# mapillary/OpenSfM

Measured on AMD Instinct MI355X. Metric: image-pairs matched/sec (+ BA LM-iters/sec, 5k cams / 500k pts), higher is better.
Workload: dtype i8 (exact int32 accumulate) + f64 RANSAC

## Files before the change

### opensfm_amd/csrc/match.hip

```cpp
#include <algorithm>
#include <cstdlib>
#include <type_traits>

#include "osfm_internal.h"

typedef int v4i __attribute__((ext_vector_type(4)));
typedef int v16i __attribute__((ext_vector_type(16)));

#ifdef OSFM_DBG_PHASES
__device__ unsigned long long g_phase[22];
#define OSFM_TICK(var) const unsigned long long var = wall_clock64();
#define OSFM_PHASE(i, t0, t1) if (threadIdx.x == 0) atomicAdd(&g_phase[i], (t1) - (t0));
extern "C" int osfm_dbg_phases(unsigned long long *out, int reset) {
  if (hipMemcpyFromSymbol(out, HIP_SYMBOL(g_phase), sizeof(g_phase)) != hipSuccess) return 1;
  if (reset) {
    unsigned long long z[22] = {};
    if (hipMemcpyToSymbol(HIP_SYMBOL(g_phase), z, sizeof(z)) != hipSuccess) return 1;
  }
  return 0;
}
#else
#define OSFM_TICK(var)
#define OSFM_PHASE(i, t0, t1)
#endif

namespace {

constexpr int kThreads = 256;
constexpr int kWaves = 4;
constexpr int kRT = 2;
constexpr int kNone = 0xFFFF;
constexpr int kCollisionD2 = 1 << 22;

__device__ __forceinline__ bool ratio_ok(int d1sq, int d2sq, double ratio) {
  if (ratio < 0.0) return (float)d1sq < (float)(-ratio) * (float)d2sq;
  const float f1 = sqrtf((float)d1sq), f2 = sqrtf((float)d2sq);
  return (double)f1 < ratio * (double)f2;
}

__device__ __forceinline__ long xcd_remap(long b, long n) {
  const long q = n >> 3, r = n & 7;
  const long xcd = b & 7, within = b >> 3;
  return (xcd < r ? xcd * (q + 1) : r * (q + 1) + (xcd - r) * q) + within;
}

struct MatchArgs {
  const int8_t *tiles;
  const int32_t *norms;
  const int32_t *hneg;
  const float *descf;
  const float *qerr;
  const int64_t *tile_off;
  const int32_t *counts;
  const int32_t *pairs;
  long n_pairs;
  double ratio;
  int symmetric;
  int query_second;
  int cap;
  int ncap;
  int32_t *out_counts;
  uint32_t *out_matches;
  int32_t *out_flags;
  long pad_tile;
  const uint32_t *bin;
  const float *seg;
  int32_t *tickets;
};
constexpr int kTicketStride = 32;

__device__ __forceinline__ void emit_matches(const MatchArgs &a, long p, int nC, const int *colBI,
                                             const unsigned short *rowres, int *misc, int tid, bool swap_halves) {
  const int lane = tid & 63, w = tid >> 6;
  int base = 0;
  for (int j0 = 0; j0 < nC; j0 += kThreads) {
    const int j = j0 + tid;
    bool m = false;
    int r = kNone;
    if (j < nC) {
      r = colBI[j];
      m = (r != kNone) && (!a.symmetric || rowres[r] == j);
    }
    const unsigned long long bal = __ballot(m);
    const int prefix = __popcll(bal & ((1ull << lane) - 1ull));
    if (lane == 0) misc[w] = __popcll(bal);
    __syncthreads();
    int woff = 0, total = 0;
#pragma unroll
    for (int w2 = 0; w2 < kWaves; ++w2) {
      const int cnt = misc[w2];
      woff += (w2 < w) ? cnt : 0;
      total += cnt;
    }
    if (m) {
      const int k = base + woff + prefix;
      if (k < a.cap) a.out_matches[p * a.cap + k] = swap_halves ? ((uint32_t)r | ((uint32_t)j << 16)) : ((uint32_t)j | ((uint32_t)r << 16));
    }
    base += total;
    __syncthreads();
  }
  if (tid == 0) a.out_counts[p] = base;
}

__device__ __forceinline__ int dot_rows8(const int8_t *tilesA, int rowA, const int8_t *tilesB, int rowB) {
  const int8_t *pa = tilesA + (long)(rowA >> 5) * OSFM_TILE_BYTES + (rowA & 31) * 16;
  const int8_t *pb = tilesB + (long)(rowB >> 5) * OSFM_TILE_BYTES + (rowB & 31) * 16;
  v4i av[8], bv[8];
#pragma unroll
  for (int q = 0; q < 8; ++q) {
    av[q] = *(const v4i *)(pa + q * 512);
    bv[q] = *(const v4i *)(pb + q * 512);
  }
  int s0 = 0, s1 = 0;
#pragma unroll
  for (int q = 0; q < 8; q += 2)
#pragma unroll
    for (int e = 0; e < 4; ++e) {
      s0 = __builtin_amdgcn_sdot4(av[q][e], bv[q][e], s0, false);
      s1 = __builtin_amdgcn_sdot4(av[q + 1][e], bv[q + 1][e], s1, false);
    }
  return s0 + s1;
}

template <class P>
__device__ __forceinline__ P *uniform_ptr(P *p) {
  const unsigned long long v = (unsigned long long)p;
  const unsigned lo = __builtin_amdgcn_readfirstlane((unsigned)v), hi = __builtin_amdgcn_readfirstlane((unsigned)(v >> 32));
  return (P *)(((unsigned long long)hi << 32) | lo);
}

__device__ __forceinline__ int wave_max(int v) {
#pragma unroll
  for (int m = 32; m >= 1; m >>= 1) v = max(v, __shfl_xor(v, m));
  return v;
}

__device__ __forceinline__ int row16_max(int x) {
  x = max(x, __builtin_amdgcn_update_dpp(x, x, 0xB1, 0xF, 0xF, false));
  x = max(x, __builtin_amdgcn_update_dpp(x, x, 0x4E, 0xF, 0xF, false));
  x = max(x, __builtin_amdgcn_update_dpp(x, x, 0x141, 0xF, 0xF, false));
  x = max(x, __builtin_amdgcn_update_dpp(x, x, 0x140, 0xF, 0xF, false));
  return x;
}

constexpr double kFqSlack = 8e-6;
__device__ __forceinline__ double fq_ratio(double ratio) { return ratio < 0.0 ? sqrt(-ratio) : ratio; }
__device__ __forceinline__ bool fq_surely_fails(int d0lo_sq, int d1hi_sq, double eps, double r) {
  const double D0lo = fmax(sqrt((double)max(d0lo_sq, 0)) - eps, 0.0) * (1.0 - kFqSlack);
  const double D1hi = (sqrt((double)max(d1hi_sq, 0)) + eps) * (1.0 + kFqSlack);
  return D0lo >= r * D1hi;
}
__device__ __forceinline__ bool fq_surely_passes(int d0hi_sq, int d1lo_sq, double eps, double r) {
  const double D0hi = (sqrt((double)max(d0hi_sq, 0)) + eps) * (1.0 + kFqSlack);
  const double D1lo = fmax(sqrt((double)max(d1lo_sq, 0)) - eps, 0.0) * (1.0 - kFqSlack);
  return D0hi < r * D1lo && D0hi < D1lo;
}
__device__ __forceinline__ float wave_minf(float v) {
#pragma unroll
  for (int m = 32; m >= 1; m >>= 1) v = fminf(v, __shfl_xor(v, m));
  return v;
}

constexpr int kCT4 = 8;
constexpr int kChunkCols4 = kCT4 * 32;
constexpr int kChunkBytes4 = kCT4 * OSFM_TILE_BYTES;

struct QueryPassShared {
  unsigned char *bbuf;
  int *hbuf;
};

template <bool GATHER, bool FQ, class Hooks>
__device__ __forceinline__ int query_pass(const QueryPassShared &sh, const int8_t *tilesQ, const int32_t *normQ, int nQ, int nslots,
                                          const unsigned short *qsel, const int8_t *tilesT, const int32_t *normT, const int32_t *hnegT,
                                          int nT, const int8_t *tiles_pad, const int32_t *hneg_pad, unsigned short *out, double ratio,
                                          int tid, const float *descQ, const float *descT, double eps, int *hit_word, int &any_hit,
                                          Hooks &&hooks) {
  asm volatile("" : "+v"(tid));
  asm volatile("" : "+s"(ratio));
  const int lane = tid & 63;
  const int w = __builtin_amdgcn_readfirstlane(tid >> 6);
  const int tT = (nT + 31) >> 5;
  const int tS = (nslots + 31) >> 5;
  const int nchunks = (tS + kCT4 - 1) / kCT4;
  const int nrb = (tT + kWaves * kRT - 1) / (kWaves * kRT);
  int flag = 0, hit = 0;

  auto dma_chunk = [&](int c) {
    unsigned char *dst = sh.bbuf + (c & 1) * kChunkBytes4;
#pragma unroll
    for (int q = 0; q < kCT4; ++q) {
      const int gt = c * kCT4 + q;
      const int8_t *src;
      if (GATHER) {
        const int slot = gt * 32 + (lane & 31);
        const int f = slot < nslots ? (int)qsel[slot] : 0;
        src = tilesQ + (long)(f >> 5) * OSFM_TILE_BYTES + w * 1024 + (lane >> 5) * 512 + (f & 31) * 16;
      } else {
        src = tilesQ + (long)(gt < tS ? gt : 0) * OSFM_TILE_BYTES + tid * 16;
      }
      __builtin_amdgcn_global_load_lds((const __attribute__((address_space(1))) void *)src,
                                       (__attribute__((address_space(3))) void *)(dst + q * OSFM_TILE_BYTES + w * 1024), 16, 0, 0);
    }
  };

  auto load_seeds = [&](int rb, int slot) {
    const int t = rb * (kWaves * kRT) + w * kRT;
    const int32_t *h0 = uniform_ptr((t < tT) ? hnegT + (long)t * 32 : hneg_pad);
    const int32_t *h1 = uniform_ptr((t + 1 < tT) ? hnegT + (long)(t + 1) * 32 : hneg_pad);
    const int32_t *hp = ((lane >> 5) ? h1 : h0) + (lane & 31);
    __builtin_amdgcn_global_load_lds((const __attribute__((address_space(1))) void *)hp,
                                     (__attribute__((address_space(3))) void *)(sh.hbuf + slot * 256 + w * 64), 4, 0, 0);
  };
  auto load_rows = [&](int rb, v4i (&af)[kRT][4], int rt) {
    const int t = rb * (kWaves * kRT) + w * kRT + rt;
    const auto *tp = (const __attribute__((address_space(1))) int8_t *)uniform_ptr((t < tT) ? tilesT + (long)t * OSFM_TILE_BYTES : tiles_pad);
#pragma unroll
    for (int ks = 0; ks < 4; ++ks) af[rt][ks] = *(const __attribute__((address_space(1))) v4i *)(tp + ks * 1024 + lane * 16);
  };
  auto load_targets = [&](int rb, v4i (&af)[kRT][4], int slot) {
    load_seeds(rb, slot);
    load_rows(rb, af, 0);
    load_rows(rb, af, 1);
  };
  v16i hn[kRT];
  auto read_seeds_rt = [&](int slot, int rt) {
#pragma unroll
    for (int g = 0; g < 4; ++g) {
      const v4i hv = *(const v4i *)(sh.hbuf + slot * 256 + w * 64 + rt * 32 + 8 * g + 4 * (lane >> 5));
      hn[rt][4 * g + 0] = hv[0];
      hn[rt][4 * g + 1] = hv[1];
      hn[rt][4 * g + 2] = hv[2];
      hn[rt][4 * g + 3] = hv[3];
    }
  };
  auto read_seeds = [&](int slot) {
    read_seeds_rt(slot, 0);
    read_seeds_rt(slot, 1);
  };

  int cb[kCT4], cs[kCT4], ci[kCT4];
  const unsigned char *bb = sh.bbuf;
  v4i bf[4];

#define OSFM_TREE_A(X, A, B)             \
  A = max(max(X[0], X[1]), X[2]);        \
  B = max(max(X[8], X[9]), X[10]);
#define OSFM_TREE_B(X, A, B)             \
  A = max(max(A, X[3]), X[4]);           \
  B = max(max(B, X[11]), X[12]);
#define OSFM_TREE_C(X, A, B)             \
  A = max(max(A, X[5]), X[6]);           \
  B = max(max(B, X[13]), X[14]);
#define OSFM_TREE_D(X, A, B, M)          \
  M = max(max(A, B), X[7]);              \
  M = max(M, X[15]);
#define OSFM_PIN __builtin_amdgcn_sched_barrier(0);

  auto step = [&](const v4i (&af)[kRT][4], v4i (&nxt)[kRT][4], int rb, int rbn, int next_slot, int t0, const unsigned char *bq) {
    const int vrb = rb;
    v16i T[3];
    int mp = 0;
    asm volatile("; osfm-step: a step of the sweep begins (tests/test_kernel_budgets_sweep.py)");
#pragma unroll
    for (int t = 0; t < kCT4; ++t) {
      if (t == 0 && t0 > 0) {
        load_targets(rbn, nxt, next_slot);
        continue;
      }
      if (t < kCT4 - 1 && t < t0) continue;
      const unsigned char *nb = (t == kCT4 - 1 ? bq + t0 * OSFM_TILE_BYTES : bq + (t + 1) * OSFM_TILE_BYTES) + lane * 16;
      v16i &C1 = T[(2 * t) % 3];
      v16i &C2 = T[(2 * t + 1) % 3];
      v16i &P2 = T[(2 * t + 2) % 3];
      int a0 = 0, b0 = 0, a1 = 0, b1 = 0, m2 = 0;
      C1 = __builtin_amdgcn_mfma_i32_32x32x32_i8(af[0][0], bf[0], hn[0], 0, 0, 0);
      OSFM_PIN
      if (t > 0) {
        OSFM_TREE_A(C2, a0, b0)
        OSFM_TREE_B(C2, a0, b0)
        OSFM_TREE_C(C2, a0, b0)
        OSFM_TREE_D(C2, a0, b0, mp)
      } else {
        load_seeds(rbn, next_slot);
      }
      OSFM_PIN
      C2 = __builtin_amdgcn_mfma_i32_32x32x32_i8(af[1][0], bf[0], hn[1], 0, 0, 0);
      OSFM_PIN
      if (t == kCT4 - 1) {
        __builtin_amdgcn_s_waitcnt(0x0F70 | (2 * kRT * 4));
        read_seeds_rt(next_slot, 0);
      }
      bf[0] = *(const v4i *)(nb);
      if (t > 0) { OSFM_TREE_A(P2, a1, b1) }
      OSFM_PIN
      C1 = __builtin_amdgcn_mfma_i32_32x32x32_i8(af[0][1], bf[1], C1, 0, 0, 0);
      OSFM_PIN
      if (t > 0) { OSFM_TREE_B(P2, a1, b1) } else { load_rows(rbn, nxt, 0); }
      if (t == kCT4 - 1) read_seeds_rt(next_slot, 1);
      OSFM_PIN
      C2 = __builtin_amdgcn_mfma_i32_32x32x32_i8(af[1][1], bf[1], C2, 0, 0, 0);
      OSFM_PIN
      bf[1] = *(const v4i *)(nb + 1024);
      if (t > 0) { OSFM_TREE_C(P2, a1, b1) }
      OSFM_PIN
      C1 = __builtin_amdgcn_mfma_i32_32x32x32_i8(af[0][2], bf[2], C1, 0, 0, 0);
      OSFM_PIN
      if (t > 0) { OSFM_TREE_D(P2, a1, b1, m2) } else { load_rows(rbn, nxt, 1); }
      OSFM_PIN
      C2 = __builtin_amdgcn_mfma_i32_32x32x32_i8(af[1][2], bf[2], C2, 0, 0, 0);
      OSFM_PIN
      bf[2] = *(const v4i *)(nb + 2048);
      if (t > 0) {
        m2 = max(m2, mp);
        asm("v_med3_i32 %0, %1, %2, %3" : "=v"(cs[t - 1]) : "v"(cb[t - 1]), "v"(m2), "v"(cs[t - 1]));
      }
      OSFM_PIN
      C1 = __builtin_amdgcn_mfma_i32_32x32x32_i8(af[0][3], bf[3], C1, 0, 0, 0);
      OSFM_PIN
      if (t > 0)
        asm volatile("v_cmp_gt_i32 vcc, %1, %2\n\ts_nop 1\n\tv_cndmask_b32 %0, %0, %3, vcc" : "+v"(ci[t - 1]) : "v"(m2), "v"(cb[t - 1]), "v"(vrb) : "vcc");
      OSFM_PIN
      C2 = __builtin_amdgcn_mfma_i32_32x32x32_i8(af[1][3], bf[3], C2, 0, 0, 0);
      OSFM_PIN
      bf[3] = *(const v4i *)(nb + 3072);
      if (t > 0) cb[t - 1] = max(cb[t - 1], m2);
      OSFM_PIN
    }
    {
      v16i &Q1 = T[(2 * (kCT4 - 1)) % 3];
      v16i &Q2 = T[(2 * (kCT4 - 1) + 1) % 3];
      int a0, b0, a1, b1, m1, m2;
      OSFM_TREE_A(Q1, a0, b0)
      OSFM_TREE_B(Q1, a0, b0)
      OSFM_TREE_C(Q1, a0, b0)
      OSFM_TREE_D(Q1, a0, b0, m1)
      OSFM_TREE_A(Q2, a1, b1)
      OSFM_TREE_B(Q2, a1, b1)
      OSFM_TREE_C(Q2, a1, b1)
      OSFM_TREE_D(Q2, a1, b1, m2)
      m2 = max(m2, m1);
      asm("v_med3_i32 %0, %1, %2, %3" : "=v"(cs[kCT4 - 1]) : "v"(cb[kCT4 - 1]), "v"(m2), "v"(cs[kCT4 - 1]));
      ci[kCT4 - 1] = m2 > cb[kCT4 - 1] ? rb : ci[kCT4 - 1];
      cb[kCT4 - 1] = max(cb[kCT4 - 1], m2);
    }
  };

  auto load_norm = [&](int c) {
    const int slot = c * kChunkCols4 + tid;
    const int f = slot < nslots ? (GATHER ? (int)qsel[slot] : slot) : -1;
    return (f >= 0 && f < nQ) ? normQ[f] : OSFM_PAD_NORM;
  };
  dma_chunk(0);
  v4i afA[kRT][4], afB[kRT][4];
  load_targets(0, afA, 0);
  int myna_next = load_norm(0);
  hooks.cold_issue();
  __builtin_amdgcn_s_waitcnt(0x0F70);
  hooks.cold_done();
  read_seeds(0);
  int sidx = 0;

  for (int c = 0; c < nchunks; ++c) {
    const int myslot = c * kChunkCols4 + tid;
    const int myf = myslot < nslots ? (GATHER ? (int)qsel[myslot] : myslot) : -1;
    const int myna = myna_next;
    __builtin_amdgcn_s_waitcnt(0x0F70);
    __syncthreads();
    bb = sh.bbuf + (c & 1) * kChunkBytes4;
    const int t0 = kCT4 - min(kCT4, tS - c * kCT4);
#pragma unroll
    for (int ks = 0; ks < 4; ++ks) bf[ks] = *(const v4i *)(bb + ks * 1024 + lane * 16);
#pragma unroll
    for (int t = 0; t < kCT4; ++t) {
      cb[t] = INT_MIN;
      cs[t] = INT_MIN;
      ci[t] = 0;
    }

    auto one_step = [&](const v4i (&cur)[kRT][4], v4i (&nxt)[kRT][4], int rb) {
      const int rbn = (rb + 1 < nrb) ? rb + 1 : 0;
      const bool live = rb * (kWaves * kRT) + w * kRT < tT;
      const int nslot = (sidx + 1) & 1;
      if (live) {
        step(cur, nxt, rb, rbn, nslot, t0, bb - t0 * OSFM_TILE_BYTES);
      } else {
        load_targets(rbn, nxt, nslot);
        __builtin_amdgcn_s_waitcnt(0x0F70);
        read_seeds(nslot);
      }
      ++sidx;
    };
    OSFM_TICK(tk0)
    hooks.chunk(c);
    if (c + 1 < nchunks) dma_chunk(c + 1);
    int rb = 0;
    for (; rb + 1 < nrb; rb += 2) {
      one_step(afA, afB, rb);
      one_step(afB, afA, rb + 1);
    }
    if (rb < nrb) {
      one_step(afA, afB, rb);
#pragma unroll
      for (int rt = 0; rt < kRT; ++rt)
#pragma unroll
        for (int ks = 0; ks < 4; ++ks) afA[rt][ks] = afB[rt][ks];
    }

    OSFM_TICK(tk1)
    if (c + 1 < nchunks) myna_next = load_norm(c + 1);
    __syncthreads();
    OSFM_TICK(tk2)
    int *scr = (int *)(sh.bbuf + (c & 1) * kChunkBytes4);
    {
      const int part = w * 2 + (lane >> 5);
#pragma unroll
      for (int t = 0; t < kCT4; ++t) {
        const int qt = (t - t0) & (kCT4 - 1);
        scr[(part * 3 + 0) * kChunkCols4 + qt * 32 + (lane & 31)] = cb[t];
        scr[(part * 3 + 1) * kChunkCols4 + qt * 32 + (lane & 31)] = cs[t];
        scr[(part * 3 + 2) * kChunkCols4 + qt * 32 + (lane & 31)] = ci[t];
      }
    }
    __syncthreads();
    int b = INT_MIN, s2 = INT_MIN, id = 0;
#pragma unroll
    for (int part = 0; part < 2 * kWaves; ++part) {
      const int pb = scr[(part * 3 + 0) * kChunkCols4 + tid], ps = scr[(part * 3 + 1) * kChunkCols4 + tid];
      const int pi = scr[(part * 3 + 2) * kChunkCols4 + tid];
      s2 = max(max(s2, ps), min(b, pb));
      id = pb > b ? (pi * 8 + part) : id;
      b = max(b, pb);
    }
    __syncthreads();
    bool want = false;
    if (myf >= 0 && myf < nQ) {
      const int d1lo = max(myna - (2 * b + 1), 0), d2hi = myna - 2 * s2;
      if (FQ) {
        want = !fq_surely_fails(d1lo, d2hi, eps, fq_ratio(ratio));
      } else {
        if (d2hi >= kCollisionD2 && ratio >= 0.0) flag = 1;
        want = ratio_ok(d1lo, d2hi, ratio);
      }
#ifdef OSFM_DBG_NORECHECK
      want = false;
#endif
      if (!want) out[myf] = kNone;
    }
    unsigned long long pending = __ballot(want);
    unsigned long long redo = 0;
    OSFM_TICK(tk3)
#ifdef OSFM_DBG_PHASES
    if (tid == 0) atomicAdd(&g_phase[(GATHER ? 5 : 0) + 4], (unsigned long long)__popcll(pending));
#endif
    while (pending) {
      int srcs[4];
#pragma unroll
      for (int g = 0; g < 4; ++g) {
        srcs[g] = pending ? (int)__builtin_ctzll(pending) : -1;
        pending &= pending - 1;
      }
      const int g = lane >> 4, sl = lane & 15;
      const int src = g == 0 ? srcs[0] : g == 1 ? srcs[1] : g == 2 ? srcs[2] : srcs[3];
      const int ssrc = src < 0 ? 0 : src;
      const int qf = __shfl(myf, ssrc), qna = __shfl(myna, ssrc), qb = __shfl(b, ssrc), qs = __shfl(s2, ssrc), qid = __shfl(id, ssrc);
      const bool tie = (qs == qb);
      const int qrb = qid >> 3, qw = (qid >> 1) & 3, qh = qid & 1;
      const int row0 = (qrb * (kWaves * kRT) + qw * kRT) * 32 + (sl & 3) + 8 * (sl >> 2) + 4 * qh, row1 = row0 + 32;
      int k0 = INT_MIN, k1 = INT_MIN;
      if (src >= 0 && !tie) {
        const bool ok0 = row0 < nT, ok1 = row1 < nT;
        const int r0 = ok0 ? row0 : 0, r1 = ok1 ? row1 : 0;
        const int8_t *pa = tilesQ + (long)(qf >> 5) * OSFM_TILE_BYTES + (qf & 31) * 16;
        const int8_t *p0 = tilesT + (long)(r0 >> 5) * OSFM_TILE_BYTES + (r0 & 31) * 16;
        const int8_t *p1 = tilesT + (long)(r1 >> 5) * OSFM_TILE_BYTES + (r1 & 31) * 16;
        v4i av[8], bv0[8], bv1[8];
#pragma unroll
        for (int q = 0; q < 8; ++q) {
          av[q] = *(const v4i *)(pa + q * 512);
          bv0[q] = *(const v4i *)(p0 + q * 512);
          bv1[q] = *(const v4i *)(p1 + q * 512);
        }
        const int n0 = normT[r0], n1 = normT[r1];
        int s0 = 0, s1 = 0;
#pragma unroll
        for (int q = 0; q < 8; ++q)
#pragma unroll
          for (int e = 0; e < 4; ++e) {
            s0 = __builtin_amdgcn_sdot4(av[q][e], bv0[q][e], s0, false);
            s1 = __builtin_amdgcn_sdot4(av[q][e], bv1[q][e], s1, false);
          }
        if (ok0) k0 = (2 * s0 - n0) * 32 + (31 - sl);
        if (ok1) k1 = (2 * s1 - n1) * 32 + (15 - sl);
      }
      const int kmax = row16_max(max(k0, k1));
      const int ksec = row16_max(k0 == kmax ? k1 : (k1 == kmax ? k0 : max(k0, k1)));
      if (src >= 0) {
        bool full = tie;
        int win = kNone;
        if (!tie) {
          const int m1 = kmax >> 5, ord = 31 - (kmax & 31);
          const int jwin = (qrb * (kWaves * kRT) + qw * kRT + (ord >> 4)) * 32 + (ord & 3) + 8 * ((ord & 15) >> 2) + 4 * qh;
          const int m2 = ksec >> 5;
          const int sa = max(m2, 2 * qs), sb = max(m2, 2 * qs + 1);
          if (FQ) {
            const double r = fq_ratio(ratio);
            if (fq_surely_passes(qna - m1, qna - sb, eps, r))
              win = jwin;
            else if (!fq_surely_fails(qna - m1, qna - sa, eps, r))
              full = true;
          } else {
            const bool ra = ratio_ok(qna - m1, qna - sa, ratio), rbb = ratio_ok(qna - m1, qna - sb, ratio);
            if (ra == rbb)
              win = ra ? jwin : kNone;
            else
              full = true;
          }
        }
        if (sl == 0 && !full) out[qf] = (unsigned short)win;
        hit |= (!full && win != kNone);
        redo |= (full && sl == 0) ? (1ull << src) : 0ull;
      }
    }
    OSFM_TICK(tk4)
    OSFM_PHASE((GATHER ? 5 : 0) + 0, tk0, tk1)
    OSFM_PHASE((GATHER ? 5 : 0) + 1, tk1, tk2)
    OSFM_PHASE((GATHER ? 5 : 0) + 2, tk2, tk3)
    OSFM_PHASE((GATHER ? 5 : 0) + 3, tk3, tk4)
    {
      unsigned lo = (unsigned)redo, hi = (unsigned)(redo >> 32);
#pragma unroll
      for (int m = 32; m >= 16; m >>= 1) {
        lo |= (unsigned)__shfl_xor((int)lo, m);
        hi |= (unsigned)__shfl_xor((int)hi, m);
      }
      redo = ((unsigned long long)(unsigned)__builtin_amdgcn_readfirstlane((int)hi) << 32) | (unsigned)__builtin_amdgcn_readfirstlane((int)lo);
    }
    if (FQ) flag += __popcll(redo);
    while (FQ && redo) {
      const int src = __builtin_ctzll(redo);
      redo &= redo - 1;
      const int qf = __shfl(myf, src), qna = __shfl(myna, src), qs2 = __shfl(s2, src);
      const double T = (sqrt((double)max(qna - 2 * qs2, 0)) + 2.0 * eps) * (1.0 + 4.0 * kFqSlack) + 1e-6;
      const double T2 = T * T;
      const int vthr = T2 >= 2.0e9 ? INT_MIN : qna - (int)T2 - 1;
      const float *qrow = descQ + (long)qf * OSFM_DESC_DIM;
      float bd0 = INFINITY, bd1 = INFINITY;
      int bi0 = INT_MAX;
      for (int i = lane; i < nT; i += 64) {
        const int v = 2 * dot_rows8(tilesQ, qf, tilesT, i) - normT[i];
        if (v >= vthr) {
          const float sq = l2sqr_rows_f32(qrow, descT + (long)i * OSFM_DESC_DIM);
          const float d = ratio < 0.0 ? sq : sqrtf(sq);
          if (d < bd1) {
            if (bd0 > d) {
              bd1 = bd0;
              bd0 = d;
              bi0 = i;
            } else {
              bd1 = d;
            }
          }
        }
      }
      const float m = wave_minf(bd0);
      const int jwin = -wave_max(bd0 == m ? -bi0 : INT_MIN);
      const float sec = wave_minf(bi0 == jwin ? bd1 : bd0);
      const bool ok = ratio < 0.0 ? (m < (float)(-ratio) * sec) : ((double)m < ratio * (double)sec);
      if (lane == 0) out[qf] = (unsigned short)(ok ? jwin : kNone);
      hit |= ok;
    }
    while (!FQ && redo) {
      const int src = __builtin_ctzll(redo);
      redo &= redo - 1;
      const int qf = __shfl(myf, src), qna = __shfl(myna, src);
      int lv = INT_MIN, lj = INT_MAX, ls = INT_MIN;
      for (int i = lane; i < nT; i += 64) {
        const int v = 2 * dot_rows8(tilesQ, qf, tilesT, i) - normT[i];
        ls = max(ls, min(lv, v));
        if (v > lv) {
          lv = v;
          lj = i;
        }
      }
      const int m1 = wave_max(lv);
      const int jwin = -wave_max(lv == m1 ? -lj : INT_MIN);
      const int m2 = wave_max(lj == jwin ? ls : lv);
      const bool ok = ratio_ok(qna - m1, qna - m2, ratio);
      if (lane == 0) out[qf] = (unsigned short)(ok ? jwin : kNone);
      hit |= ok;
    }
  }
  if (hit) *hit_word = 1;
  __syncthreads();
  any_hit = *hit_word;
  return flag;
}

struct PairRange {
  long first;
  int len;
};
__device__ __forceinline__ PairRange pair_range(long n_pairs, int x) {
  const long q = n_pairs >> 3, r = n_pairs & 7;
  return PairRange{x < r ? x * (q + 1) : r * (q + 1) + (x - r) * q, (int)(q + (x < r ? 1 : 0))};
}
__device__ __forceinline__ int draw_pair(const MatchArgs &a, int xcd, int *hdr, bool have, int t) {
  for (int k = hdr[8]; k < 8; ++k) {
    const int x = (xcd + k) & 7;
    const PairRange r = pair_range(a.n_pairs, x);
    if (!have) t = atomicAdd(a.tickets + x * kTicketStride, 1);
    have = false;
    if (t < r.len) {
      hdr[8] = k;
      return (int)(r.first + t);
    }
  }
  hdr[8] = 8;
  return -1;
}
__device__ __forceinline__ void finish_pair_header(const MatchArgs &a, int *hdr) {
  const int img1 = hdr[1], img2 = hdr[2];
  const int n1 = a.counts[img1], n2 = a.counts[img2];
  const int o1 = (int)a.tile_off[img1], o2 = (int)a.tile_off[img2];
  hdr[3] = n1;
  hdr[4] = n2;
  hdr[5] = o1;
  hdr[6] = o2;
  hdr[7] = 1;
}
__device__ __forceinline__ void fetch_pair_header(const MatchArgs &a, int xcd, int *hdr) {
  const int p = draw_pair(a, xcd, hdr, false, 0);
  hdr[0] = p;
  hdr[7] = 1;
  if (p >= 0) {
    const int img1 = a.pairs[2 * (long)p], img2 = a.pairs[2 * (long)p + 1];
    hdr[1] = img1;
    hdr[2] = img2;
    finish_pair_header(a, hdr);
  }
}
struct NextPairFetch {
  const MatchArgs &a;
  int xcd;
  int *hdr;
  int tid;
  int t;
  __device__ __forceinline__ void cold_issue() {
    if (tid == 0) {
      const int k = hdr[8];
      t = k < 8 ? atomicAdd(a.tickets + ((xcd + k) & 7) * kTicketStride, 1) : 0;
    }
  }
  __device__ __forceinline__ void cold_done() {
    if (tid == 0) {
      hdr[0] = draw_pair(a, xcd, hdr, hdr[8] < 8, t);
      hdr[7] = 0;
    }
  }
  __device__ __forceinline__ void chunk(int c) {
    if (c > 1 || __builtin_amdgcn_readfirstlane(tid >> 6) != 0) return;
    const int pn = __builtin_amdgcn_readfirstlane(hdr[0]);
    if (pn < 0) return;
    if (c == 0) {
      if (tid < 2)
        __builtin_amdgcn_global_load_lds((const __attribute__((address_space(1))) void *)(a.pairs + 2 * (long)pn + tid),
                                         (__attribute__((address_space(3))) void *)(hdr + 1), 4, 0, 0);
    } else if (tid < 4) {
      const int img = hdr[1 + (tid & 1)];
      const int32_t *src = tid < 2 ? a.counts + img : (const int32_t *)(a.tile_off + img);
      __builtin_amdgcn_global_load_lds((const __attribute__((address_space(1))) void *)src,
                                       (__attribute__((address_space(3))) void *)(hdr + 3), 4, 0, 0);
      if (tid == 0) hdr[7] = 1;
    }
  }
};
struct NoFetch {
  __device__ __forceinline__ void cold_issue() {}
  __device__ __forceinline__ void cold_done() {}
  __device__ __forceinline__ void chunk(int) {}
};

__device__ __forceinline__ int fresh_tid(int wave) {
  int t = wave * 64 + (int)__builtin_amdgcn_mbcnt_hi(~0u, __builtin_amdgcn_mbcnt_lo(~0u, 0u));
  asm volatile("" : "+v"(t));
  return t;
}

template <bool FQ>
__global__ void __launch_bounds__(kThreads, 2) match_fused_kernel(MatchArgs a) {
  extern __shared__ __attribute__((aligned(16))) unsigned char smem[];
  QueryPassShared sh;
  sh.bbuf = smem;
  sh.hbuf = (int *)(smem + 2 * kChunkBytes4);
  int *misc = (int *)(smem + 2 * kChunkBytes4) + 2 * kChunkCols4;
  int *hdr = misc + 16;
  unsigned short *resA = (unsigned short *)(hdr + 16);
  unsigned short *resB = resA + a.ncap;
  unsigned short *cand = resB + a.ncap;

  const int xcd = blockIdx.x & 7;
  const int8_t *tiles_pad = a.tiles + a.pad_tile * OSFM_TILE_BYTES;
  const int32_t *hneg_pad = a.hneg + a.pad_tile * 32;
  OSFM_TICK(tw0)
#ifdef OSFM_DBG_PHASES
  unsigned long long t_prev = tw0;
#endif
  const int wave = __builtin_amdgcn_readfirstlane(threadIdx.x >> 6);
  if (threadIdx.x == 0) {
    hdr[8] = 0;
    fetch_pair_header(a, xcd, hdr);
  }
  __syncthreads();
  for (;;) {
  const int tid = fresh_tid(wave);
  const long p = __builtin_amdgcn_readfirstlane(hdr[0]);
  if (p < 0) break;
  if (__builtin_amdgcn_readfirstlane(hdr[7]) == 0) {
    __syncthreads();
    if (tid == 0) finish_pair_header(a, hdr);
    __syncthreads();
  }
  const int img1 = __builtin_amdgcn_readfirstlane(hdr[1]), img2 = __builtin_amdgcn_readfirstlane(hdr[2]);
  const int n1 = __builtin_amdgcn_readfirstlane(hdr[3]), n2 = __builtin_amdgcn_readfirstlane(hdr[4]);
  const long off1 = __builtin_amdgcn_readfirstlane(hdr[5]), off2 = __builtin_amdgcn_readfirstlane(hdr[6]);
  if (tid == 0) {
    misc[8] = 0;
    misc[9] = 0;
    misc[10] = 0;
  }
  __syncthreads();
  if (n1 < 2 || n2 < 2) {
    if (tid == 0) {
      a.out_counts[p] = 0;
      a.out_flags[p] = 0;
      fetch_pair_header(a, xcd, hdr);
    }
    __syncthreads();
#ifdef OSFM_DBG_PHASES
    {
      OSFM_TICK(te)
      OSFM_PHASE(19, t_prev, te)
      if (threadIdx.x == 0) atomicAdd(&g_phase[20], 1ull);
      t_prev = te;
    }
#endif
    continue;
  }
  const bool rows_second = a.symmetric || a.query_second;
  const int imgA = rows_second ? img2 : img1, imgB = rows_second ? img1 : img2;
  const int nA = rows_second ? n2 : n1, nB = rows_second ? n1 : n2;
  const long offA = rows_second ? off2 : off1, offB = rows_second ? off1 : off2;
  const int8_t *tilesA = a.tiles + offA * OSFM_TILE_BYTES;
  const int8_t *tilesB = a.tiles + offB * OSFM_TILE_BYTES;
  const int32_t *normA = a.norms + offA * 32;
  const int32_t *normB = a.norms + offB * 32;
  const int32_t *hnegA = a.hneg + offA * 32;
  const int32_t *hnegB = a.hneg + offB * 32;
  OSFM_TICK(tq0)
  const float *descA = FQ ? a.descf + offA * (long)(32 * OSFM_DESC_DIM) : nullptr;
  const float *descB = FQ ? a.descf + offB * (long)(32 * OSFM_DESC_DIM) : nullptr;
  const double eps = FQ ? (double)a.qerr[imgA] + (double)a.qerr[imgB] : 0.0;
  int any = 0;
  auto flush_flag = [&](int f) {
    if (FQ) {
      if ((fresh_tid(wave) & 63) == 0 && f) atomicAdd(&misc[8], f);
    } else if (f) {
      misc[8] = 1;
    }
  };
  int flag = query_pass<false, FQ>(sh, tilesA, normA, nA, nA, nullptr, tilesB, normB, hnegB, nB, tiles_pad, hneg_pad, resA, a.ratio, fresh_tid(wave),
                                   descA, descB, eps, misc + 9, any, NextPairFetch{a, xcd, hdr, fresh_tid(wave), 0});
  OSFM_TICK(tq1)
  OSFM_PHASE(10, tq0, tq1)
  if (a.symmetric && any) {
    const int tid = fresh_tid(wave), lane = tid & 63, w = tid >> 6;
    for (int j = tid; j < nB; j += kThreads) resB[j] = kNone;
    __syncthreads();
    for (int q = tid; q < nA; q += kThreads) {
      const int b = resA[q];
      if (b != kNone) resB[b] = 0;
    }
    __syncthreads();
    int base = 0;
    for (int j0 = 0; j0 < nB; j0 += kThreads) {
      const int j = j0 + tid;
      const bool m = j < nB && resB[j] == 0;
      const unsigned long long bal = __ballot(m);
      if (lane == 0) misc[w] = __popcll(bal);
      __syncthreads();
      int woff = 0, total = 0;
#pragma unroll
      for (int w2 = 0; w2 < kWaves; ++w2) {
        const int cnt = misc[w2];
        woff += (w2 < w) ? cnt : 0;
        total += cnt;
      }
      if (m) {
        cand[base + woff + __popcll(bal & ((1ull << lane) - 1ull))] = (unsigned short)j;
        resB[j] = kNone;
      }
      base += total;
      __syncthreads();
    }
    const int nK = base;
    OSFM_TICK(tq2)
    OSFM_PHASE(11, tq1, tq2)
    flush_flag(flag);
    flag = query_pass<true, FQ>(sh, tilesB, normB, nB, nK, cand, tilesA, normA, hnegA, nA, tiles_pad, hneg_pad, resB, a.ratio, fresh_tid(wave), descB, descA,
                                 eps, misc + 10, any, NoFetch{});
  }
  OSFM_TICK(tq3)
  OSFM_PHASE(12, tq1, tq3)
  flush_flag(flag);
  __builtin_amdgcn_s_waitcnt(0x0F70);
  __syncthreads();
  if (fresh_tid(wave) == 0) a.out_flags[p] = misc[8];
  if (!any) {
    if (fresh_tid(wave) == 0) a.out_counts[p] = 0;
  } else {
    const int tid = fresh_tid(wave), lane = tid & 63, w = tid >> 6;
    const bool qs = !a.symmetric && a.query_second;
    const unsigned short *res1 = a.symmetric ? resB : resA;
    const unsigned short *res2 = a.symmetric ? resA : nullptr;
    const int nE = qs ? n2 : n1;
    int base = 0;
    for (int j0 = 0; j0 < nE; j0 += kThreads) {
      const int j = j0 + tid;
      bool m = false;
      int r = kNone;
      if (j < nE) {
        r = res1[j];
        m = (r != kNone) && (!res2 || res2[r] == j);
      }
      const unsigned long long bal = __ballot(m);
      const int prefix = __popcll(bal & ((1ull << lane) - 1ull));
      if (lane == 0) misc[w] = __popcll(bal);
      __syncthreads();
      int woff = 0, total = 0;
#pragma unroll
      for (int w2 = 0; w2 < kWaves; ++w2) {
        const int cnt = misc[w2];
        woff += (w2 < w) ? cnt : 0;
        total += cnt;
      }
      if (m) {
        const int k = base + woff + prefix;
        if (k < a.cap) a.out_matches[p * a.cap + k] = qs ? ((uint32_t)r | ((uint32_t)j << 16)) : ((uint32_t)j | ((uint32_t)r << 16));
      }
      base += total;
      __syncthreads();
    }
    if (tid == 0) a.out_counts[p] = base;
  }
  OSFM_TICK(tq4)
  OSFM_PHASE(13, tq3, tq4)
  OSFM_PHASE(14, tq0, tq4)
#ifdef OSFM_DBG_PHASES
  if (threadIdx.x == 0) atomicAdd(&g_phase[15], 1ull);
  OSFM_PHASE(16, t_prev, tq0)
  t_prev = tq4;
#endif
  }
#ifdef OSFM_DBG_PHASES
  if (threadIdx.x == 0) {
    atomicAdd(&g_phase[17], wall_clock64() - tw0);
    atomicAdd(&g_phase[18], 1ull);
  }
#endif
}

__device__ __forceinline__ void load_row(const int8_t *tiles, int row, v4i out[8]) {
  const int8_t *t = tiles + (long)(row >> 5) * OSFM_TILE_BYTES + (row & 31) * 16;
#pragma unroll
  for (int ks = 0; ks < 4; ++ks) {
    out[2 * ks] = *(const v4i *)(t + ks * 1024);
    out[2 * ks + 1] = *(const v4i *)(t + ks * 1024 + 512);
  }
}

__device__ void exact_direction(const int8_t *tilesQ, const int32_t *normQ, int nQ, const int8_t *tilesT,
                                const int32_t *normT, int nT, double ratio, int tid, int *res_int,
                                unsigned short *res_u16, const float *segQ, const float *segT) {
  for (int q = tid; q < nQ; q += kThreads) {
    v4i qa[8];
    load_row(tilesQ, q, qa);
    const int nq = normQ[q];
    const float sq = segQ ? segQ[q] : 0.f;
    float bd0 = INFINITY, bd1 = INFINITY;
    int bi0 = kNone;
    for (int t = 0; t < nT; ++t) {
      v4i ta[8];
      load_row(tilesT, t, ta);
      int sdot = 0;
#pragma unroll
      for (int k = 0; k < 8; ++k)
#pragma unroll
        for (int e = 0; e < 4; ++e) sdot = __builtin_amdgcn_sdot4(qa[k][e], ta[k][e], sdot, false);
      const int d2i = nq + normT[t] - 2 * sdot;
      float d2f = (float)d2i;
      if (segQ) {
        const float ts = sq - segT[t];
        const float tt = ts * ts;
        d2f = d2f + tt;
      }
      const float d = ratio < 0.0 ? d2f : sqrtf(d2f);
      if (d < bd1) {
        if (bd0 > d) {
          bd1 = bd0;
          bd0 = d;
          bi0 = t;
        } else {
          bd1 = d;
        }
      }
    }
    const bool ok = ratio < 0.0 ? (bd0 < (float)(-ratio) * bd1) : ((double)bd0 < ratio * (double)bd1);
    const int v = ok ? bi0 : kNone;
    if (res_int) res_int[q] = v;
    if (res_u16) res_u16[q] = (unsigned short)v;
  }
}

__global__ void __launch_bounds__(kThreads) match_exact_kernel(MatchArgs a, int only_flagged) {
  extern __shared__ __attribute__((aligned(16))) unsigned char smem[];
  int *colBI = (int *)smem;
  unsigned short *rowres = (unsigned short *)(colBI + a.ncap);
  int *misc = (int *)(rowres + a.ncap);
  const int tid = threadIdx.x;
  const long p = blockIdx.x;
  if (only_flagged && a.out_flags[p] == 0) return;
  const bool qs = !a.symmetric && a.query_second;
  const int imgC = a.pairs[2 * p + (qs ? 1 : 0)], imgR = a.pairs[2 * p + (qs ? 0 : 1)];
  const int nC = a.counts[imgC], nR = a.counts[imgR];
  if (nC < 2 || nR < 2) {
    if (tid == 0) a.out_counts[p] = 0;
    return;
  }
  const int8_t *tilesC = a.tiles + a.tile_off[imgC] * OSFM_TILE_BYTES;
  const int8_t *tilesR = a.tiles + a.tile_off[imgR] * OSFM_TILE_BYTES;
  const int32_t *normC = a.norms + a.tile_off[imgC] * 32;
  const int32_t *normR = a.norms + a.tile_off[imgR] * 32;
  const float *segC = a.seg ? a.seg + a.tile_off[imgC] * 32 : nullptr, *segR = a.seg ? a.seg + a.tile_off[imgR] * 32 : nullptr;
  exact_direction(tilesC, normC, nC, tilesR, normR, nR, a.ratio, tid, colBI, nullptr, segC, segR);
  if (a.symmetric) exact_direction(tilesR, normR, nR, tilesC, normC, nC, a.ratio, tid, nullptr, rowres, segR, segC);
  __syncthreads();
  emit_matches(a, p, nC, colBI, rowres, misc, tid, qs);
}

constexpr int kFloatTileFloats = 32 * OSFM_DESC_DIM;

__device__ void float_direction(const float *descQ, int nQ, const float *descT, int nT, double ratio, int tid, float *stage, int *res_int,
                                unsigned short *res_u16) {
  const int tT = (nT + 31) >> 5;
  for (int q0 = 0; q0 < nQ; q0 += kThreads) {
    const int q = q0 + tid;
    const bool live = q < nQ;
    float qa[OSFM_DESC_DIM];
#pragma unroll
    for (int k4 = 0; k4 < OSFM_DESC_DIM; k4 += 4) {
      float4 v = make_float4(0.f, 0.f, 0.f, 0.f);
      if (live) v = *(const float4 *)(descQ + (size_t)q * OSFM_DESC_DIM + k4);
      qa[k4] = v.x;
      qa[k4 + 1] = v.y;
      qa[k4 + 2] = v.z;
      qa[k4 + 3] = v.w;
    }
    float bd0 = INFINITY, bd1 = INFINITY;
    int bi0 = kNone;
    for (int tt = 0; tt < tT; ++tt) {
      __syncthreads();
      for (int k = tid * 4; k < kFloatTileFloats; k += kThreads * 4) *(float4 *)(stage + k) = *(const float4 *)(descT + (size_t)tt * kFloatTileFloats + k);
      __syncthreads();
      const int nt = min(32, nT - tt * 32);
      for (int t = 0; t < nt; ++t) {
        const float *b = stage + t * OSFM_DESC_DIM;
        float acc[4][8];
#pragma unroll
        for (int v = 0; v < 4; ++v)
#pragma unroll
          for (int l = 0; l < 8; ++l) acc[v][l] = 0.f;
#pragma unroll
        for (int jb = 0; jb < OSFM_DESC_DIM; jb += 32)
#pragma unroll
          for (int v = 0; v < 4; ++v)
#pragma unroll
            for (int l4 = 0; l4 < 8; l4 += 4) {
              const float4 c = *(const float4 *)(b + jb + 8 * v + l4);
              const float cc[4] = {c.x, c.y, c.z, c.w};
#pragma unroll
              for (int e = 0; e < 4; ++e) {
                const float d = qa[jb + 8 * v + l4 + e] - cc[e];
                const float sq = d * d;
                acc[v][l4 + e] = acc[v][l4 + e] + sq;
              }
            }
        float sv[8];
#pragma unroll
        for (int l = 0; l < 8; ++l) sv[l] = (acc[0][l] + acc[1][l]) + (acc[2][l] + acc[3][l]);
        const float sqd = ((sv[0] + sv[1]) + (sv[2] + sv[3])) + ((sv[4] + sv[5]) + (sv[6] + sv[7]));
        const float d = ratio < 0.0 ? sqd : sqrtf(sqd);
        if (d < bd1) {
          if (bd0 > d) {
            bd1 = bd0;
            bd0 = d;
            bi0 = tt * 32 + t;
          } else {
            bd1 = d;
          }
        }
      }
    }
    if (live) {
      const bool ok = ratio < 0.0 ? (bd0 < (float)(-ratio) * bd1) : ((double)bd0 < ratio * (double)bd1);
      const int v = ok ? bi0 : kNone;
      if (res_int) res_int[q] = v;
      if (res_u16) res_u16[q] = (unsigned short)v;
    }
  }
}

__global__ void __launch_bounds__(kThreads) match_float_kernel(MatchArgs a) {
  extern __shared__ __attribute__((aligned(16))) unsigned char smem[];
  float *stage = (float *)smem;
  int *colBI = (int *)(stage + kFloatTileFloats);
  unsigned short *rowres = (unsigned short *)(colBI + a.ncap);
  int *misc = (int *)(rowres + a.ncap);
  const int tid = threadIdx.x;
  const long p = blockIdx.x;
  if (tid == 0 && a.out_flags) a.out_flags[p] = 0;
  const bool qs = !a.symmetric && a.query_second;
  const int imgC = a.pairs[2 * p + (qs ? 1 : 0)], imgR = a.pairs[2 * p + (qs ? 0 : 1)];
  const int nC = a.counts[imgC], nR = a.counts[imgR];
  if (nC < 2 || nR < 2) {
    if (tid == 0) a.out_counts[p] = 0;
    return;
  }
  const float *descC = a.descf + a.tile_off[imgC] * kFloatTileFloats;
  const float *descR = a.descf + a.tile_off[imgR] * kFloatTileFloats;
  float_direction(descC, nC, descR, nR, a.ratio, tid, stage, colBI, nullptr);
  if (a.symmetric) float_direction(descR, nR, descC, nC, a.ratio, tid, stage, nullptr, rowres);
  __syncthreads();
  emit_matches(a, p, nC, colBI, rowres, misc, tid, qs);
}

constexpr int kHamStageRows = 256;

__device__ void hamming_direction(const uint32_t *binQ, int nQ, const uint32_t *binT, int nT, double ratio, int tid, uint32_t *stage, int *res_int,
                                  unsigned short *res_u16) {
  for (int q0 = 0; q0 < nQ; q0 += kThreads) {
    const int q = q0 + tid;
    const bool live = q < nQ;
    uint4 qa[4];
#pragma unroll
    for (int k = 0; k < 4; ++k) qa[k] = live ? *(const uint4 *)(binQ + (size_t)q * 16 + 4 * k) : make_uint4(0u, 0u, 0u, 0u);
    int bd0 = 0x7fffffff, bd1 = 0x7fffffff, bi0 = kNone;
    for (int t0 = 0; t0 < nT; t0 += kHamStageRows) {
      const int nt = min(kHamStageRows, nT - t0);
      __syncthreads();
      for (int k = tid; k < nt * 4; k += kThreads) *(uint4 *)(stage + 4 * k) = *(const uint4 *)(binT + (size_t)t0 * 16 + 4 * k);
      __syncthreads();
      for (int t = 0; t < nt; ++t) {
        const uint4 *b = (const uint4 *)(stage + t * 16);
        int d = 0;
#pragma unroll
        for (int k = 0; k < 4; ++k) {
          const uint4 c = b[k];
          d += __popc(qa[k].x ^ c.x) + __popc(qa[k].y ^ c.y) + __popc(qa[k].z ^ c.z) + __popc(qa[k].w ^ c.w);
        }
        if (d < bd1) {
          if (bd0 > d) {
            bd1 = bd0;
            bd0 = d;
            bi0 = t0 + t;
          } else {
            bd1 = d;
          }
        }
      }
    }
    if (live) {
      const bool ok = (double)(float)bd0 < ratio * (double)(float)bd1;
      const int v = ok ? bi0 : kNone;
      if (res_int) res_int[q] = v;
      if (res_u16) res_u16[q] = (unsigned short)v;
    }
  }
}

__global__ void __launch_bounds__(kThreads) match_hamming_kernel(MatchArgs a) {
  extern __shared__ __attribute__((aligned(16))) unsigned char smem[];
  uint32_t *stage = (uint32_t *)smem;
  int *colBI = (int *)(stage + kHamStageRows * 16);
  unsigned short *rowres = (unsigned short *)(colBI + a.ncap);
  int *misc = (int *)(rowres + a.ncap);
  const int tid = threadIdx.x;
  const long p = blockIdx.x;
  if (tid == 0 && a.out_flags) a.out_flags[p] = 0;
  const bool qs = !a.symmetric && a.query_second;
  const int imgC = a.pairs[2 * p + (qs ? 1 : 0)], imgR = a.pairs[2 * p + (qs ? 0 : 1)];
  const int nC = a.counts[imgC], nR = a.counts[imgR];
  if (nC < 2 || nR < 2) {
    if (tid == 0) a.out_counts[p] = 0;
    return;
  }
  const uint32_t *binC = a.bin + a.tile_off[imgC] * (32 * 16);
  const uint32_t *binR = a.bin + a.tile_off[imgR] * (32 * 16);
  hamming_direction(binC, nC, binR, nR, a.ratio, tid, stage, colBI, nullptr);
  if (a.symmetric) hamming_direction(binR, nR, binC, nC, a.ratio, tid, stage, nullptr, rowres);
  __syncthreads();
  emit_matches(a, p, nC, colBI, rowres, misc, tid, qs);
}

}

size_t osfm_match_lds_bytes(int ncap) { return (size_t)2 * kChunkBytes4 + 2 * kChunkCols4 * 4 + 128 + (size_t)ncap * 6; }

static int ensure_kernel_attributes(int device) {
  static OsfmPerDeviceOnce once;
  return once.run(device, []() -> int {
    OSFM_HIP(hipFuncSetAttribute((const void *)match_fused_kernel<false>, hipFuncAttributeMaxDynamicSharedMemorySize, 160 * 1024));
    OSFM_HIP(hipFuncSetAttribute((const void *)match_fused_kernel<true>, hipFuncAttributeMaxDynamicSharedMemorySize, 160 * 1024));
    OSFM_HIP(hipFuncSetAttribute((const void *)match_exact_kernel, hipFuncAttributeMaxDynamicSharedMemorySize, 160 * 1024));
    OSFM_HIP(hipFuncSetAttribute((const void *)match_float_kernel, hipFuncAttributeMaxDynamicSharedMemorySize, 160 * 1024));
    OSFM_HIP(hipFuncSetAttribute((const void *)match_hamming_kernel, hipFuncAttributeMaxDynamicSharedMemorySize, 160 * 1024));
    return OSFM_OK;
  });
}

int osfm_launch_match(osfm_ctx *ctx, const osfm_store *store, const int32_t *d_pairs, int64_t n_pairs,
                      double ratio, int symmetric, int squared_ratio, int cap, int32_t *d_counts, uint32_t *d_matches,
                      int32_t *d_flags, bool exact_kernel, hipStream_t stream) {
  if (n_pairs == 0) return OSFM_OK;
  MatchArgs a;
  a.tiles = store->d_tiles;
  a.norms = store->d_norms;
  a.hneg = store->d_hneg;
  a.descf = store->d_descf;
  a.qerr = store->d_qerr;
  a.seg = store->d_seg;
  a.bin = store->d_bin;
  a.tile_off = store->d_tile_off;
  a.counts = store->d_counts;
  a.pairs = d_pairs;
  a.n_pairs = n_pairs;
  a.ratio = squared_ratio ? -(double)(float)(ratio * ratio) : ratio;
  a.symmetric = symmetric;
  a.query_second = squared_ratio && !symmetric;
  a.cap = cap;
  a.ncap = ((store->max_count + 127) / 128) * 128;
  if (a.ncap < 128) a.ncap = 128;
  a.out_counts = d_counts;
  a.out_matches = d_matches;
  a.out_flags = d_flags;
  a.pad_tile = store->tile_off[store->n_images];
  a.tickets = nullptr;
  OSFM_REQUIRE(a.ncap <= OSFM_MAX_FEATURES, OSFM_E_UNSUPPORTED, "more than %d features in an image", OSFM_MAX_FEATURES);
  OSFM_REQUIRE(n_pairs < (1ll << 31), OSFM_E_INVALID, "too many pairs in one launch");
  OSFM_TRY(ensure_kernel_attributes(ctx->device));
  const bool fused = !store->is_binary && !store->d_seg && !exact_kernel && (!store->is_float || store->quantised);
  unsigned resident = 0;
  if (fused) {
    OSFM_REQUIRE(a.pad_tile < (1ll << 31), OSFM_E_UNSUPPORTED, "too many tiles in the store");
    OSFM_REQUIRE(ctx->num_cus > 0, OSFM_E_INVALID, "the context knows no compute units");
    if (!ctx->d_match_tickets) OSFM_HIP(hipMalloc(&ctx->d_match_tickets, 8 * kTicketStride * sizeof(int32_t)));
    OSFM_HIP(hipMemsetAsync(ctx->d_match_tickets, 0, 8 * kTicketStride * sizeof(int32_t), stream));
    a.tickets = (int32_t *)ctx->d_match_tickets;
    resident = (unsigned)std::min<int64_t>(n_pairs, 2 * (int64_t)ctx->num_cus);
  }
  if (store->is_binary) {
    if (squared_ratio) a.ratio = ratio * ratio;
    if (exact_kernel && d_flags != nullptr) return OSFM_OK;
    const size_t lds = (size_t)kHamStageRows * 64 + (size_t)a.ncap * 6 + 64;
    hipLaunchKernelGGL(match_hamming_kernel, dim3((unsigned)n_pairs), dim3(kThreads), lds, stream, a);
  } else if (store->d_seg) {
    if (exact_kernel && d_flags != nullptr) return OSFM_OK;
    if (d_flags) OSFM_HIP(hipMemsetAsync(d_flags, 0, (size_t)n_pairs * sizeof(int32_t), stream));
    const size_t lds = (size_t)a.ncap * 6 + 64;
    hipLaunchKernelGGL(match_exact_kernel, dim3((unsigned)n_pairs), dim3(kThreads), lds, stream, a, 0);
  } else if (store->is_float) {
    if (exact_kernel && d_flags != nullptr) return OSFM_OK;
    if (!exact_kernel && store->quantised) {
      hipLaunchKernelGGL(match_fused_kernel<true>, dim3(resident), dim3(kThreads), osfm_match_lds_bytes(a.ncap), stream, a);
    } else {
      if (d_flags) OSFM_HIP(hipMemsetAsync(d_flags, 0, (size_t)n_pairs * sizeof(int32_t), stream));
      const size_t lds = (size_t)kFloatTileFloats * sizeof(float) + (size_t)a.ncap * 6 + 64;
      hipLaunchKernelGGL(match_float_kernel, dim3((unsigned)n_pairs), dim3(kThreads), lds, stream, a);
    }
  } else if (!exact_kernel) {
    hipLaunchKernelGGL(match_fused_kernel<false>, dim3(resident), dim3(kThreads), osfm_match_lds_bytes(a.ncap), stream, a);
  } else {
    const size_t lds = (size_t)a.ncap * 6 + 64;
    hipLaunchKernelGGL(match_exact_kernel, dim3((unsigned)n_pairs), dim3(kThreads), lds, stream, a, d_flags != nullptr ? 1 : 0);
  }
  OSFM_HIP(hipGetLastError());
  return OSFM_OK;
}
```

Baseline: 2.677 million.

## Pack row-block index into low bits of best-score key, drop separate index array

The running best and second-best scores are now stored as keys with the row block index shifted into the low six bits. This removes the separate ci index array, its compare-and-select in the MFMA inner step, one of three scratch stores per tile, and one __syncthreads in the reduction. The index is decoded from the winning key afterwards. It also zeroes misc through an opaque register and restricts a waitcnt to wave 0. The approach relies on the score shifted left by six bits not overflowing int32, and ties between equal scores now resolve by row block rather than by first occurrence.

```diff
diff --git a/opensfm_amd/csrc/match.hip b/opensfm_amd/csrc/match.hip
--- a/opensfm_amd/csrc/match.hip
+++ b/opensfm_amd/csrc/match.hip
@@ -164,6 +164,10 @@
 constexpr int kCT4 = 8;
 constexpr int kChunkCols4 = kCT4 * 32;
 constexpr int kChunkBytes4 = kCT4 * OSFM_TILE_BYTES;
+constexpr int kKeyShift = 6;
+static_assert(((OSFM_MAX_FEATURES + 31) / 32 + kWaves * kRT - 1) / (kWaves * kRT) <= (1 << kKeyShift),
+              "a row block index of the largest image does not fit the class key");
+__device__ __forceinline__ int class_key(int u, int rb) { return (int)(((unsigned)u << kKeyShift) + (unsigned)rb); }
 
 struct QueryPassShared {
   unsigned char *bbuf;
@@ -239,7 +243,7 @@
     read_seeds_rt(slot, 1);
   };
 
-  int cb[kCT4], cs[kCT4], ci[kCT4];
+  int cb[kCT4], cs[kCT4];
   const unsigned char *bb = sh.bbuf;
   v4i bf[4];
 
@@ -255,10 +259,12 @@
 #define OSFM_TREE_D(X, A, B, M)          \
   M = max(max(A, B), X[7]);              \
   M = max(M, X[15]);
+#define OSFM_TREE_DX(X, A, B, M, E)      \
+  M = max(max(A, B), X[7]);              \
+  M = max(max(M, X[15]), E);
 #define OSFM_PIN __builtin_amdgcn_sched_barrier(0);
 
   auto step = [&](const v4i (&af)[kRT][4], v4i (&nxt)[kRT][4], int rb, int rbn, int next_slot, int t0, const unsigned char *bq) {
-    const int vrb = rb;
     v16i T[3];
     int mp = 0;
     asm volatile("; osfm-step: a step of the sweep begins (tests/test_kernel_budgets_sweep.py)");
@@ -306,20 +312,18 @@
       OSFM_PIN
       C1 = __builtin_amdgcn_mfma_i32_32x32x32_i8(af[0][2], bf[2], C1, 0, 0, 0);
       OSFM_PIN
-      if (t > 0) { OSFM_TREE_D(P2, a1, b1, m2) } else { load_rows(rbn, nxt, 1); }
+      if (t > 0) { OSFM_TREE_DX(P2, a1, b1, m2, mp) } else { load_rows(rbn, nxt, 1); }
       OSFM_PIN
       C2 = __builtin_amdgcn_mfma_i32_32x32x32_i8(af[1][2], bf[2], C2, 0, 0, 0);
       OSFM_PIN
       bf[2] = *(const v4i *)(nb + 2048);
       if (t > 0) {
-        m2 = max(m2, mp);
+        m2 = class_key(m2, rb);
         asm("v_med3_i32 %0, %1, %2, %3" : "=v"(cs[t - 1]) : "v"(cb[t - 1]), "v"(m2), "v"(cs[t - 1]));
       }
       OSFM_PIN
       C1 = __builtin_amdgcn_mfma_i32_32x32x32_i8(af[0][3], bf[3], C1, 0, 0, 0);
       OSFM_PIN
-      if (t > 0)
-        asm volatile("v_cmp_gt_i32 vcc, %1, %2\n\ts_nop 1\n\tv_cndmask_b32 %0, %0, %3, vcc" : "+v"(ci[t - 1]) : "v"(m2), "v"(cb[t - 1]), "v"(vrb) : "vcc");
       OSFM_PIN
       C2 = __builtin_amdgcn_mfma_i32_32x32x32_i8(af[1][3], bf[3], C2, 0, 0, 0);
       OSFM_PIN
@@ -338,10 +342,9 @@
       OSFM_TREE_A(Q2, a1, b1)
       OSFM_TREE_B(Q2, a1, b1)
       OSFM_TREE_C(Q2, a1, b1)
-      OSFM_TREE_D(Q2, a1, b1, m2)
-      m2 = max(m2, m1);
+      OSFM_TREE_DX(Q2, a1, b1, m2, m1)
+      m2 = class_key(m2, rb);
       asm("v_med3_i32 %0, %1, %2, %3" : "=v"(cs[kCT4 - 1]) : "v"(cb[kCT4 - 1]), "v"(m2), "v"(cs[kCT4 - 1]));
-      ci[kCT4 - 1] = m2 > cb[kCT4 - 1] ? rb : ci[kCT4 - 1];
       cb[kCT4 - 1] = max(cb[kCT4 - 1], m2);
     }
   };
@@ -375,7 +378,6 @@
     for (int t = 0; t < kCT4; ++t) {
       cb[t] = INT_MIN;
       cs[t] = INT_MIN;
-      ci[t] = 0;
     }
 
     auto one_step = [&](const v4i (&cur)[kRT][4], v4i (&nxt)[kRT][4], int rb) {
@@ -417,22 +419,20 @@
 #pragma unroll
       for (int t = 0; t < kCT4; ++t) {
         const int qt = (t - t0) & (kCT4 - 1);
-        scr[(part * 3 + 0) * kChunkCols4 + qt * 32 + (lane & 31)] = cb[t];
-        scr[(part * 3 + 1) * kChunkCols4 + qt * 32 + (lane & 31)] = cs[t];
-        scr[(part * 3 + 2) * kChunkCols4 + qt * 32 + (lane & 31)] = ci[t];
+        scr[(part * 2 + 0) * kChunkCols4 + qt * 32 + (lane & 31)] = cb[t];
+        scr[(part * 2 + 1) * kChunkCols4 + qt * 32 + (lane & 31)] = cs[t];
       }
     }
     __syncthreads();
-    int b = INT_MIN, s2 = INT_MIN, id = 0;
+    int kb = INT_MIN, ks = INT_MIN, wpart = 0;
 #pragma unroll
     for (int part = 0; part < 2 * kWaves; ++part) {
-      const int pb = scr[(part * 3 + 0) * kChunkCols4 + tid], ps = scr[(part * 3 + 1) * kChunkCols4 + tid];
-      const int pi = scr[(part * 3 + 2) * kChunkCols4 + tid];
-      s2 = max(max(s2, ps), min(b, pb));
-      id = pb > b ? (pi * 8 + part) : id;
-      b = max(b, pb);
-    }
-    __syncthreads();
+      const int pb = scr[(part * 2 + 0) * kChunkCols4 + tid], ps = scr[(part * 2 + 1) * kChunkCols4 + tid];
+      ks = max(max(ks, ps), min(kb, pb));
+      wpart = pb > kb ? part : wpart;
+      kb = max(kb, pb);
+    }
+    const int b = kb >> kKeyShift, s2 = ks >> kKeyShift, id = (kb & ((1 << kKeyShift) - 1)) * 8 + wpart;
     bool want = false;
     if (myf >= 0 && myf < nQ) {
       const int d1lo = max(myna - (2 * b + 1), 0), d2hi = myna - 2 * s2;
@@ -725,9 +725,11 @@
   const int n1 = __builtin_amdgcn_readfirstlane(hdr[3]), n2 = __builtin_amdgcn_readfirstlane(hdr[4]);
   const long off1 = __builtin_amdgcn_readfirstlane(hdr[5]), off2 = __builtin_amdgcn_readfirstlane(hdr[6]);
   if (tid == 0) {
-    misc[8] = 0;
-    misc[9] = 0;
-    misc[10] = 0;
+    int zero = 0;
+    asm volatile("" : "+v"(zero));
+    misc[8] = zero;
+    misc[9] = zero;
+    misc[10] = zero;
   }
   __syncthreads();
   if (n1 < 2 || n2 < 2) {
@@ -813,7 +815,7 @@
   OSFM_TICK(tq3)
   OSFM_PHASE(12, tq1, tq3)
   flush_flag(flag);
-  __builtin_amdgcn_s_waitcnt(0x0F70);
+  if (wave == 0) __builtin_amdgcn_s_waitcnt(0x0F70);
   __syncthreads();
   if (fresh_tid(wave) == 0) a.out_flags[p] = misc[8];
   if (!any) {
```

Result: no change. 2.684 million (median of 6 runs) (+0.3%).
